# ishine/zerovox.cpp

Measured on AMD Instinct MI355X. Metric: audio-seconds/wall-second (xRT) end-to-end phoneme->22.05 kHz wav, higher is better.
Workload: dtype f16*f16->f32 (MFMA) convs, f32 (MFMA) attention/linear, f32 activations

## Files before the change

zerovox.cpp_amd/csrc/conv_gemm.hip:

```cpp
#include "kernels.h"
#include "knobs.h"
#include "mfma_common.h"

namespace zv
{

__device__ __forceinline__ int gemm_groups_dev(int Cout_p) { return ((Cout_p + 31) >> 5) >> 3; }

__device__ __forceinline__ int conv_gemm_units_dev(int Cin_p, int K)
{
    const int full = Cin_p >> 8, rem = Cin_p & 255;
    return K * (full * 4 + ((rem + 63) >> 6));
}

size_t conv_gemm_weight_halfs(int Cin_p, int Cout_p, int K)
{
    return (size_t)conv_gemm_tiles(Cout_p) * conv_gemm_units(Cin_p, K) * 2048;
}

typedef unsigned int u32x4s __attribute__((ext_vector_type(4)));
__device__ __forceinline__ void dma_piece(u32x4s rsrc, unsigned lds_base, unsigned voff)
{
    unsigned keep;
    asm volatile("s_mov_b32 %0, m0\n\ts_mov_b32 m0, %1\n\ts_nop 4\n\tbuffer_load_dwordx4 %2, %3, 0 offen lds\n\ts_mov_b32 m0, %0"
                 : "=&s"(keep)
                 : "s"(lds_base), "v"(voff), "s"(rsrc)
                 : "memory");
}

__device__ __forceinline__ u32x4s make_rsrc(const void *base, unsigned bytes)
{
    const uint64_t a = (uint64_t)base;
    u32x4s r;
    r[0] = __builtin_amdgcn_readfirstlane((unsigned)a);
    r[1] = __builtin_amdgcn_readfirstlane((unsigned)(a >> 32) & 0xFFFFu);
    r[2] = __builtin_amdgcn_readfirstlane(bytes);
    r[3] = 0x00020000u;
    return r;
}

void pack_conv_weight_gemm(const uint16_t *w, int K, int IC, int OC, int Cin_p, int Cout_p, uint16_t *dst)
{
    const int ng = conv_gemm_groups(Cout_p), nu = conv_gemm_units(Cin_p, K), ntk = conv_gemm_tiles(Cout_p);
    size_t gbase = 0;
    for (int g = 0; g < ng; g++)
    {
        const int ntg = (g == ng - 1) ? ntk - 8 * g : 8;
        int u = 0;
        for (int c0 = 0; c0 < Cin_p; c0 += 256)
        {
            const int nsub = (std::min(256, Cin_p - c0) + 63) / 64;
            for (int tap = 0; tap < K; tap++)
                for (int sub = 0; sub < nsub; sub++, u++)
                    for (int hf = 0; hf < 2; hf++)
                        for (int nt = 0; nt < ntg; nt++)
                            for (int wt = 0; wt < 2; wt++)
                            {
                                uint16_t *d = dst + gbase + ((((size_t)u * 2 + hf) * ntg + nt) * 2 + wt) * 512;
                                for (int lane = 0; lane < 64; lane++)
                                    for (int j = 0; j < 8; j++)
                                    {
                                        const int oc = (g * 8 + nt) * 32 + 2 * (lane & 15) + wt;
                                        const int ic = c0 + sub * 64 + hf * 32 + 8 * (lane >> 4) + j;
                                        d[lane * 8 + j] = (oc < OC && ic < IC) ? w[((size_t)oc * IC + ic) * K + tap] : (uint16_t)0;
                                    }
                            }
        }
        gbase += (size_t)nu * 4 * ntg * 512;
    }
}

template <bool EXTRA>
__device__ __forceinline__ void conv_gemm_body(const ConvJobs &jobs, const int g, const int rt)
{
    constexpr int BM = 256, UNIT = 32768;
    constexpr int ntg = EXTRA ? 9 : 8;
    constexpr int AH = 16384, BH = ntg * 2048;
    constexpr int SLOT = AH + 18432;
    const ConvJob &J = jobs.j[0];
    const int useg = rt / jobs.tps;
    const Seg sg = seg_at(jobs.segs, useg);
    const int L = sg.rows * jobs.rate;
    const int m0 = (rt - useg * jobs.tps) * BM;
    if (m0 >= L) return;
    const size_t row0 = (size_t)sg.row0 * jobs.rate;

    extern __shared__ __attribute__((aligned(1024))) char smem[];
    const unsigned lds0 = (unsigned)(uintptr_t)smem;
    const int tid = threadIdx.x, lane = tid & 63;
    const int wave = __builtin_amdgcn_readfirstlane(tid >> 6);
    const int wm = wave >> 2, wn = wave & 3;
    const int lc = lane & 15, lg = lane >> 4;
    const int K = J.K, dil = J.dil, Cin_p = J.Cin_p, ldx = J.ldx;
    const int nunits = conv_gemm_units_dev(Cin_p, K), nhalf = 2 * nunits;
    constexpr int bunit = ntg * 4096;

    const u32x4s rs_a = make_rsrc((const _Float16 *)J.x0 + row0 * ldx, (unsigned)((size_t)L * ldx * 2));
    const u32x4s rs_b = make_rsrc((const char *)J.w8 + (size_t)g * nunits * UNIT, (unsigned)((size_t)nunits * bunit));

    int a_voff[2];
#pragma unroll
    for (int i = 0; i < 2; i++)
    {
        const int row = (wave * 2 + i) * 16 + (lane >> 2);
        const int piece = (lane & 3) ^ ((row >> 1) & 3);
        a_voff[i] = ((m0 - J.pad + row) * ldx + piece * 8) * 2;
    }

    int uc0 = 0, utap = 0, usub = 0, unsub = (min(256, Cin_p) + 63) >> 6, uh = 0;
    unsigned i_abase = 0;
    int i_aoff = 0, i_boff = 0;
    auto issue_begin = [&](int h) {
        i_abase = lds0 + (h & 3) * SLOT;
        i_aoff = (utap * dil * ldx + uc0 + usub * 64 + uh * 32) * 2;
        i_boff = (h >> 1) * bunit + (h & 1) * BH;
        if (++uh == 2)
        {
            uh = 0;
            if (++usub == unsub)
            {
                usub = 0;
                if (++utap == K)
                {
                    utap = 0;
                    uc0 += 256;
                    unsub = (min(256, Cin_p - uc0) + 63) >> 6;
                }
            }
        }
    };
    auto issue_pa = [&](int i) { dma_piece(rs_a, i_abase + (wave * 2 + i) * 1024, (unsigned)(a_voff[i] + i_aoff)); };
    auto issue_pb = [&](int i) { dma_piece(rs_b, i_abase + AH + (wave * 2 + i) * 1024, (unsigned)(i_boff + (wave * 2 + i) * 1024 + lane * 16)); };
    auto issue_part = [&](int i) {
        issue_pa(i);
        issue_pb(i);
    };
    auto issue_x = [&]() {
        if (EXTRA && wave < 2) dma_piece(rs_b, i_abase + AH + (16 + wave) * 1024, (unsigned)(i_boff + (16 + wave) * 1024 + lane * 16));
    };
    const bool five = EXTRA && wave < 2;

    const int swz = (lc >> 1) & 3;
    const int a_rd = (wm * 128 + lc) * 64 + ((lg ^ swz) << 4);
    const int ax_rd = (wave * 32 + lc) * 64 + ((lg ^ swz) << 4);
    const int b_rd = AH + wn * 4096 + lane * 16;

    floatx4 acc[8][4];
    floatx4 accx[2][2];
    if (wave >= 4) __builtin_amdgcn_s_setprio(1);
#pragma unroll
    for (int h = 0; h < 3; h++)
        if (h < nhalf)
        {
            issue_begin(h);
            issue_part(0);
            issue_part(1);
            issue_x();
        }
    half8 aA[4], bb[4], axA, bxb[2];
#define ZV_G16_READ0(hn)                                                                                          \
    {                                                                                                             \
        const char *nb_ = smem + ((hn) & 3) * SLOT;                                                               \
        _Pragma("unroll") for (int tm = 0; tm < 4; tm++) aA[tm] = *(const half8 *)(nb_ + a_rd + tm * 1024);       \
        _Pragma("unroll") for (int tn = 0; tn < 4; tn++) bb[tn] = *(const half8 *)(nb_ + b_rd + tn * 1024);       \
        if constexpr (EXTRA)                                                                                      \
        {                                                                                                         \
            axA = *(const half8 *)(nb_ + ax_rd);                                                                  \
            bxb[0] = *(const half8 *)(nb_ + AH + 16 * 1024 + lane * 16);                                          \
            bxb[1] = *(const half8 *)(nb_ + AH + 17 * 1024 + lane * 16);                                          \
        }                                                                                                         \
    }
    {
        if (nhalf > 2)
        {
            if (five) asm volatile("s_waitcnt vmcnt(5)" ::: "memory");
            else asm volatile("s_waitcnt vmcnt(4)" ::: "memory");
        }
        else
            asm volatile("s_waitcnt vmcnt(0)" ::: "memory");
        __syncthreads();
        ZV_G16_READ0(0)
    }
    const floatx4 zero4 = {0.f, 0.f, 0.f, 0.f};
    for (int h = 0; h < nhalf; h++)
    {
        if (h > 0)
        {
            if (h + 2 < nhalf)
            {
                if (five) asm volatile("s_waitcnt vmcnt(5)" ::: "memory");
                else asm volatile("s_waitcnt vmcnt(4)" ::: "memory");
            }
            else
                asm volatile("s_waitcnt vmcnt(0)" ::: "memory");
            __syncthreads();
        }
// ... 128 lines not shown
                    v0 = lrelu(v0, J.oslope);
                    v1 = lrelu(v1, J.oslope);
                }
                outv[0][hf][i] = v0;
                outv[1][hf][i] = v1;
                if (t < L)
                {
                    const float2v o = {v0, v1};
                    __builtin_nontemporal_store(o, (float2v *)(out + (size_t)t * J.ldo + oc));
                }
            }
        if (J.stat_part && oc < J.stat_C && blk * 32 < L)
        {
#pragma unroll
            for (int ch = 0; ch < 2; ch++)
            {
                double s1 = 0.0, s2 = 0.0;
#pragma unroll
                for (int st = 0; st < 4; st++)
                {
                    if (st)
                    {
                        s1 = __shfl_xor(s1, 32, 64);
                        s2 = __shfl_xor(s2, 32, 64);
                    }
                    if ((lg >> 1) == (st & 1))
#pragma unroll
                        for (int i = 0; i < 4; i++)
                        {
                            const int t = t_first + 16 * (st >> 1) + 4 * lg + i;
                            const double x = (t < L) ? (double)outv[ch][st >> 1][i] : 0.0;
                            s1 += x;
                            s2 += x * x;
                        }
                }
                s1 += __shfl_xor(s1, 16, 64);
                s2 += __shfl_xor(s2, 16, 64);
                if (lg == 2) *(double2 *)(J.stat_part + (((size_t)useg * J.stat_nblk + blk) * J.stat_C + oc + ch) * 2) = make_double2(s1, s2);
            }
        }
    };
    const int tbase = m0 + wm * 128;
#pragma unroll
    for (int p = 0; p < 2; p++)
#pragma unroll
        for (int b4 = 0; b4 < 4; b4++)
            finish_block(acc[2 * b4][2 * p], acc[2 * b4][2 * p + 1], acc[2 * b4 + 1][2 * p], acc[2 * b4 + 1][2 * p + 1], tbase + b4 * 32,
                         ((g * 8 + wn * 2 + p) << 5) + 2 * lc, (m0 >> 5) + wm * 4 + b4);
    if constexpr (EXTRA)
        finish_block(accx[0][0], accx[0][1], accx[1][0], accx[1][1], m0 + wave * 32, ((g * 8 + 8) << 5) + 2 * lc, (m0 >> 5) + wave);
}

__global__ __launch_bounds__(512, 2) void conv_gemm_kernel(const ConvJobs jobs)
{
    const ConvJob &J = jobs.j[0];
    const int ng = (gemm_groups_dev(J.Cout_p));
    const int rts = jobs.tps * jobs.segs.nseg;
    int g, rt;
    if (jobs.order == 2 && ng > 1)
    {
        if ((int)blockIdx.x < rts) { g = ng - 1; rt = blockIdx.x; }
        else { const int b2 = blockIdx.x - rts; g = b2 % (ng - 1); rt = b2 / (ng - 1); }
    }
    else
    {
        g = blockIdx.x % ng;
        rt = blockIdx.x / ng;
    }
    if (rt >= rts) return;
    const bool ninth = g == ng - 1 && ((J.Cout_p + 31) >> 5) - 8 * ng == 1;
    if (ninth)
        conv_gemm_body<true>(jobs, g, rt);
    else
        conv_gemm_body<false>(jobs, g, rt);
}

hipError_t launch_conv_gemm(hipStream_t s, const ConvJob &job, const Segs &segs, int rate)
{
    const ConvGemmPlan p = conv_gemm_plan(job.Cout_p, ConvCall{1, segs.nseg, segs.max_rows, rate, 0, 0});
    if (job.stat_part && job.stat_nblk * 32 < segs.max_rows * rate) return hipErrorInvalidValue;
    ConvJobs js;
    js.j[0] = job;
    js.j[0].dbg = diag_bits();
    for (int i = 1; i < CONV_MAX_JOBS; i++) js.j[i] = js.j[0];
    js.segs = segs;
    js.rate = rate;
    js.nt_begin = 0;
    js.order = p.order;
    js.tps = p.tps;
    return launch_lds(conv_gemm_kernel, dim3(p.gx, 1, 1), dim3(p.threads), p.lds_bytes, s, js);
}

}
```

zerovox.cpp_amd/csrc/conv_plan.h:

```cpp
#pragma once

#include <stddef.h>

#include "conv_xcd.h"
#include "knobs.h"
#include "tile_deal.h"

namespace zv
{

constexpr long BATCH_ROWS = 16384;
inline bool batch_switch(int value, bool picked_by_itself) { return value != 0 && (value == 2 || picked_by_itself); }
inline bool batch_rows(long rows) { return rows >= BATCH_ROWS; }

constexpr size_t LDS_PER_WG = 160 * 1024;
constexpr size_t LDS_TWO_WGS = 80 * 1024;
constexpr size_t LDS_DEFAULT = 64 * 1024;

inline int plan_round_up(int x, int a) { return (x + a - 1) / a * a; }

inline int &conv_packed_utts()
{
    static thread_local int n = 0;
    return n;
}
struct ConvPackedUtts
{
    int saved;
    explicit ConvPackedUtts(int n) : saved(conv_packed_utts()) { conv_packed_utts() = n; }
    ~ConvPackedUtts() { conv_packed_utts() = saved; }
    ConvPackedUtts(const ConvPackedUtts &) = delete;
    ConvPackedUtts &operator=(const ConvPackedUtts &) = delete;
};

struct ConvCall
{
    int njobs, nseg, max_rows, rate, n_cu, nt_begin;
    int nutt = conv_packed_utts();
};
inline bool conv_call_is_batch(const ConvCall &c) { return c.nseg > 1 || c.nutt > 1; }

inline int conv_gemm_groups(int Cout_p) { return ((Cout_p + 31) / 32) / 8; }
inline int conv_gemm_tiles(int Cout_p)
{
    const int nt = (Cout_p + 31) / 32, ng = nt / 8;
    return ng * 8 + ((nt - ng * 8 == 1 && ng >= 1) ? 1 : 0);
}
inline int conv_gemm_units(int Cin_p, int K)
{
    int n = 0;
    for (int c0 = 0; c0 < Cin_p; c0 += 256) n += K * (((Cin_p - c0 < 256 ? Cin_p - c0 : 256) + 63) / 64);
    return n;
}

enum ConvPrologue : int
{
    PRO_RAW_F16 = 0,
    PRO_ACT = 1,
    PRO_NORM_ACT = 2,
    PRO_MELNORM = 3,
    PRO_SUM3_ACT = 4,
    PRO_SCALE_ACT = 5
};

#ifndef ZV_SINGLE_LW
#define ZV_SINGLE_LW 4
#endif
#ifndef ZV_CONV_BATCH_ROUTE
#define ZV_CONV_BATCH_ROUTE 1
#endif

struct ConvDesc
{
    int  K, dil, pad, Cin_p, Cout_p, ck, pro, ldx;
    bool has_w8, out_f16, has_res, has_stat, eact, three_inputs;
};

inline bool conv_gemm_takes(const ConvDesc &j, const ConvCall &c)
{
    const long rows = (long)c.max_rows * c.rate * c.nseg;
    return batch_switch(knob(ZV_CONV_GEMM), batch_rows(rows)) && j.has_w8 && j.pro == PRO_RAW_F16 && j.Cin_p >= 128 &&
           conv_gemm_groups(j.Cout_p) >= 1 && !j.out_f16 && (j.ldx & 7) == 0;
}

struct ConvGemmPlan
{
    int    order, tps, gx, threads;
    size_t lds_bytes;
};
inline ConvGemmPlan conv_gemm_plan(int Cout_p, const ConvCall &c)
{
    ConvGemmPlan p{};
    p.order = knob(ZV_GEMM_ORDER);
    p.tps = (c.max_rows * c.rate + 255) / 256;
    const int ng = conv_gemm_groups(Cout_p), rts = p.tps * c.nseg;
    p.gx = (p.order == 1 && (ng == 1 || ng == 2 || ng == 4)) ? plan_round_up(rts, 8 / ng) * ng : rts * ng;
    p.threads = 512;
    p.lds_bytes = 4 * (16384 + 18432);
    return p;
}

inline bool conv_stream_ok(const ConvDesc &j, const ConvCall &c)
{
    return c.njobs == 1 && c.nt_begin == 0 && (j.pro == PRO_ACT || j.pro == PRO_SCALE_ACT) && j.K == 3 && j.dil == 1 && j.pad == 1 &&
           (j.Cin_p == 64 || j.Cin_p == 128) && j.ck == j.Cin_p && (j.ldx & 3) == 0 && !j.has_res && !j.has_stat && !j.eact && !j.out_f16 &&
           !j.three_inputs;
}

inline bool conv_tiled_exists(int MT, int WN, int NT)
{
    return (NT == 1 && (MT == 1 || MT == 2 || MT == 4) && (WN == 1 || WN == 2 || WN == 4)) || (NT == 2 && MT == 2 && WN == 4);
}

enum ConvForm { CONV_STREAM, CONV_LOADER, CONV_TILED };
struct ConvPlan
{
    bool     valid;
    ConvForm form;
    int      MT, WN, NT;
    int      strip, nkc;
    int      tps;
    int      gx, gy, gz, threads;
    size_t   lds_bytes;
    int      tile_bytes;
    int      xcd_nx, xcd_ny, xcd_spread;
    int      warm;
};

inline bool conv_plan_tiles(ConvPlan &p, bool loader, int MT, int WN, int NT, int Lmax, int ntiles, int halo, int ck, int dmax, const ConvCall &c)
{
    const int BM = 32 * MT * (4 / WN);
    p.form = loader ? CONV_LOADER : CONV_TILED;
    p.MT = MT, p.WN = WN, p.NT = NT;
    p.tps = (Lmax + BM - 1) / BM;
    p.gx = p.tps * c.nseg, p.gy = (ntiles + WN * NT - 1) / (WN * NT), p.gz = c.njobs;
// ... 272 lines not shown
```

zerovox.cpp_amd/csrc/kernels.h:

```cpp
#pragma once

#include <hip/hip_runtime.h>
#include <stdint.h>

#include "conv_plan.h"
#include "voc_plan.h"
#include "stage_plan.h"
#include "level.h"

#ifdef ZV_DIAG
#define ZV_DBGBITS(x) (x)
#else
#define ZV_DBGBITS(x) 0
#endif

namespace zv
{

__host__ __device__ static inline int round_up(int x, int a) { return (x + a - 1) / a * a; }

struct Seg
{
    int32_t row0, rows;
    int32_t aux;
    int32_t pad;
};
struct Segs
{
    const Seg *tab;
    int        nseg;
    int        max_rows;
    Seg        one;
};
__host__ __device__ static inline Seg seg_at(const Segs &s, int u)
{
    Seg g = s.tab ? s.tab[u] : s.one;
#if defined(__HIP_DEVICE_COMPILE__)
    g.row0 = __builtin_amdgcn_readfirstlane(g.row0);
    g.rows = __builtin_amdgcn_readfirstlane(g.rows);
    g.aux = __builtin_amdgcn_readfirstlane(g.aux);
#endif
    return g;
}
static inline Segs segs_single(int rows, int aux = 0)
{
    Segs s;
    s.tab = nullptr;
    s.nseg = 1;
    s.max_rows = rows;
    s.one.row0 = 0;
    s.one.rows = rows;
    s.one.aux = aux;
    s.one.pad = 0;
    return s;
}


struct ConvJob
{
    const void  *x0, *x1, *x2;
    int          ldx;
    int          pro;
    float        slope, pscale;
    const float *pa, *pb;
    const float *pstat;
    int          L, Cin_p, Cout_p, K, dil, pad;
    int          ck;
    const void  *w;
    const void  *w8;
    const float *bias;
    const float *res;
    int          ldres;
    float        escale;
    int          eact;
    float        oslope;
    int          out_f16;
    void        *out;
    int          ldo;
    int          dbg;
    int          pstat_seg, pab_seg;
    double      *stat_part;
    int          stat_nblk, stat_C;
};

constexpr int CONV_MAX_JOBS = 4;
struct ConvJobs
{
    ConvJob j[CONV_MAX_JOBS];
    Segs    segs;
    int     rate;
    int     tps;
    int     nt_begin;
    int     order;
    int     tile_bytes;
    int     xcd_ny, xcd_nx;
    int     xcd_spread;
    int     warm;
#ifdef ZV_STAMPS
    unsigned long long *stamp;
#endif
};

size_t packed_conv_weight_halfs(int Cin_p, int Cout_p, int K);
int    conv_pick_ck(int Cin_p, int ck_max = 0);
void   pack_conv_weight(const uint16_t *w, int K, int IC, int OC, int Cin_p, int Cout_p, int ck, uint16_t *dst);
size_t conv_gemm_weight_halfs(int Cin_p, int Cout_p, int K);
void   pack_conv_weight_gemm(const uint16_t *w, int K, int IC, int OC, int Cin_p, int Cout_p, uint16_t *dst);
hipError_t launch_conv(hipStream_t s, const ConvJob *jobs, int njobs, int n_cu, const Segs &segs, int rate);

struct PairJob
{
    const float *y;
    float       *out;
    const void  *w1, *w2;
    const void  *w1r, *w2r;
    const float *b1, *b2;
    int          L, Cp, K, dil;
    float        slope;
    int          dbg;
    const float *sum_in;
    float       *sum_out;
};
constexpr int PAIR_MAX_JOBS = 3;
struct PairJobs
{
    PairJob j[PAIR_MAX_JOBS];
    Segs    segs;
    int     rate;
    int     njobs, kmax;
    int     deal_c;
#ifdef ZV_STAMPS
    unsigned long long *stamp;
#endif
    float  *merge_out;
    int     ring_off;
};
size_t     pair_weight_halfs(int Cp, int K);
void       pack_pair_weight(const uint16_t *w, int K, int C, int Cp, uint16_t *dst);
size_t     pair_weight16_halfs(int Cp, int K);
void       pack_pair_weight16(const uint16_t *w, int K, int C, int Cp, uint16_t *dst, bool conv2_layout);
size_t     pair_ring_weight_halfs(int Cp, int K);
void       pack_pair_weight_ring(const uint16_t *w, int K, int C, int Cp, uint16_t *dst, bool conv2_layout);
hipError_t launch_pair(hipStream_t s, const PairJob *jobs, int njobs, int n_cu, const Segs &segs, int rate, float *merge_out = nullptr);

struct TripleJob
{
    const float *y;
    float       *out;
    const void  *w1[TRIPLE_MAX_DIL], *w2[TRIPLE_MAX_DIL];
    const void  *w1x[TRIPLE_MAX_DIL], *w2x[TRIPLE_MAX_DIL];
    const float *b1[TRIPLE_MAX_DIL], *b2[TRIPLE_MAX_DIL];
    int          dil[TRIPLE_MAX_DIL];
// ... 106 lines not shown
```

zerovox.cpp_amd/csrc/knobs.h:

```cpp
#pragma once

namespace zv
{

#define ZV_KNOB_LIST(X)                                                                                                               \
    X(ZV_NO_FUSE, 0)                                                                  \
    X(ZV_NO_TRIPLE, 0)                                                                          \
    X(ZV_FUSE256, 0)                                                \
    X(ZV_NO_MERGE, 0)                                                               \
    X(ZV_MERGE_ALWAYS, 0)                 \
    X(ZV_MERGE_SEQ, 1)          \
    X(ZV_MERGE_MAXC, 256)                                  \
    X(ZV_TAIL_GROUPS, 8)                                                        \
    X(ZV_ARENA_FILL, 0)                                         \
    X(ZV_DEC_PREPASS, -1)                                      \
    X(ZV_CONV_MT, 0)                                                              \
    X(ZV_CONV_NT, 0)                                                     \
    X(ZV_CONV_SINGLE, 1)                                    \
    X(ZV_CONV_GEMM, 1)                  \
    X(ZV_CONV_STREAM, 1)        \
    X(ZV_VOC_RUNS, 1)           \
    X(ZV_DEC_RUNS, 1)           \
    X(ZV_DEC_PACK, 1)           \
    X(ZV_UP_GEMM, 1)           \
    X(ZV_GEMM_ORDER, 2)         \
    X(ZV_PAIR_MT, 0)                                                                  \
    X(ZV_CONV_XCD, 1)           \
    X(ZV_CONV_WARM, 1)          \
    X(ZV_LINEAR_MERGED, 1)      \
    X(ZV_BLOCK64, 3)            \
    X(ZV_PAIR64_RING, 1)               \
    X(ZV_TRIPLE_V2, 1)                               \
    X(ZV_TRIPLE_DB, 1)                                                                     \
    X(ZV_TRIPLE_INTERLEAVE, 1)                                                               \
    X(ZV_ATT_SCALAR, 0)                                                                               \
    X(ZV_ATT_MFMA, 0)                                                          \
    X(ZV_LN_TAIL, 1)

#ifdef ZV_DIAG
#define ZV_KNOB_LIST_DIAG(X)                                                                                                          \
    X(ZV_DBG, 0)                                                                       \
    X(ZV_LDS_PAD, 0)            \
    X(ZV_STAMP_CP, 0)                               \
    X(ZV_STAMP_CONV, 0)                                    \
    X(ZV_STAMP_CIN, 0)
#else
#define ZV_KNOB_LIST_DIAG(X)
#endif

enum Knob : int
{
#define ZV_KNOB_ENUM(n, d) n,
    ZV_KNOB_LIST(ZV_KNOB_ENUM)
    ZV_KNOB_LIST_DIAG(ZV_KNOB_ENUM)
#undef ZV_KNOB_ENUM
    ZV_KNOB_COUNT
};

int         knob(Knob k);
bool        knob_set(const char *name, int value);
void        knob_reset();
bool        knob_get(const char *name, int *value);
unsigned    knob_epoch();
const char *knob_name(int k);
#ifdef ZV_DIAG
inline int diag_bits() { return knob(ZV_DBG); }
#else
inline int diag_bits() { return 0; }
#endif

}
```

zerovox.cpp_amd/csrc/model.cpp:

```cpp
#include "schedule.h"

#include <algorithm>

namespace zv
{

Model::~Model()
{
    hipSetDevice(device);
    for (Lane &l : lanes_) hipStreamSynchronize(l.stream);
    drop_graphs();
    prof_clear();
    for (void *p : allocs_) hipFree(p);
    for (hipEvent_t e : batch_events_)
        if (e) hipEventDestroy(e);
    for (Lane &l : lanes_)
    {
        if (l.copy_stream) hipStreamSynchronize(l.copy_stream);
        if (l.arena.base) hipFree(l.arena.base);
        if (l.io) hipFree(l.io);
        if (l.pinned) hipHostFree(l.pinned);
        for (hipEvent_t e : l.tail_events) hipEventDestroy(e);
        if (l.copy_stream) hipStreamDestroy(l.copy_stream);
        if (l.stream) hipStreamDestroy(l.stream);
// ... 120 lines not shown
    ZV_HIP(hipStreamSynchronize(stream()));
    drop_graphs();
    DeviceArena &ar = lane().arena;
    if (ar.base) hipFree(ar.base);
    ar = DeviceArena();
    lane().runs_tab = nullptr;
    lane().runs_n = 0;
    void *p = nullptr;
    if (hipMalloc(&p, bytes) != hipSuccess) fail(ZV_ERR_OOM, "hipMalloc(%zu) for the activation arena failed", bytes);
    const int fill = knob(ZV_ARENA_FILL);
    ZV_HIP(hipMemsetAsync(p, fill, bytes, stream()));
    ar = DeviceArena{(char *)p, bytes, 0};
}

void Model::reserve(uint32_t max_phonemes, uint32_t max_frames) { reserve_batch(Batch::single(std::max(1u, max_phonemes), std::max(1u, max_frames), 1)); }

void Model::reserve_batch(const Batch &b) { arena_require(arena_bytes_for(b)); }


void Model::prof_clear()
{
    for (auto &p : prof)
    {
        hipEventDestroy(p.e0);
        hipEventDestroy(p.e1);
    }
    prof.clear();
}

void Model::tick(hipEvent_t *e0)
{
    *e0 = nullptr;
    if (!profiling || in_group_) return;
    ZV_HIP(hipEventCreate(e0));
    ZV_HIP(hipEventRecord(*e0, stream()));
}

void Model::tock(hipEvent_t e0, const char *name, double bytes, double flops)
{
    if (!profiling) return;
    if (in_group_)
    {
        group_bytes_ += bytes;
        group_flops_ += flops;
        group_n_++;
        return;
    }
    hipEvent_t e1;
    ZV_HIP(hipEventCreate(&e1));
    ZV_HIP(hipEventRecord(e1, stream()));
    prof.push_back({name, e0, e1, bytes, flops, group_n_ > 0 ? group_n_ : 1});
}

void Model::group_begin()
{
    if (!profiling) return;
    ZV_HIP(hipEventCreate(&group_e0_));
    ZV_HIP(hipEventRecord(group_e0_, stream()));
    in_group_ = true;
    group_bytes_ = group_flops_ = 0.0;
    group_n_ = 0;
}

void Model::group_end(const char *name)
{
    if (!profiling || !in_group_) return;
    in_group_ = false;
    tock(group_e0_, name, group_bytes_, group_flops_);
    group_n_ = 0;
}

ConvJob Model::job(const ConvW &w) const
{
    ConvJob j;
    memset(&j, 0, sizeof(j));
    j.Cin_p = w.Cin_p;
    j.Cout_p = w.Cout_p;
    j.K = w.K;
    j.dil = 1;
    j.pad = (w.K - 1) / 2;
    j.ck = w.ck;
    j.w = w.w;
    j.w8 = w.w8;
    j.bias = w.bias;
    j.pro = PRO_ACT;
    j.slope = 1.0f;
    j.pscale = 1.0f;
    j.escale = 1.0f;
    j.ldx = w.Cin_p;
    j.ldo = w.Cout_p;
    return j;
}

void Model::dbg_inject(void *dev, int ld, int cols, size_t rows)
{
    ZV_HIP(hipMemcpy2DAsync(dev, (size_t)ld * 4, dbg_layer.x, (size_t)cols * 4, (size_t)cols * 4, rows, hipMemcpyHostToDevice, stream()));
}

void Model::dbg_extract(const void *dev, int ld, int cols, size_t rows)
{
    ZV_HIP(hipMemcpy2DAsync(dbg_layer.out, (size_t)cols * 4, dev, (size_t)ld * 4, (size_t)cols * 4, rows, hipMemcpyDeviceToHost, stream()));
    ZV_HIP(hipStreamSynchronize(stream()));
    dbg_layer.done = true;
}

void Model::conv(const ConvJob *jobs, int n, const Segs &segs, int rate, const char *name, double bytes, double flops)
{
    ZV_LAUNCH(name, bytes, flops, launch_conv(stream(), jobs, n, n_cu, segs, rate));
}

void Model::drop_graphs()
{
    sync_all_lanes();
    for (auto &g : graphs_)
        if (g.exec) hipGraphExecDestroy(g.exec);
    graphs_.clear();
}

template <typename F> void Model::run_captured(int kind, const Batch &b, const void *const (&key)[CapturedGraph::NKEY], F &&enqueue)
{
    for (auto &g : graphs_)
        if (g.kind == kind && g.epoch == knob_epoch() && b.same_schedule(g.b) && memcmp(g.p, key, sizeof(key)) == 0)
        {
            ZV_HIP(hipGraphLaunch(g.exec, stream()));
            lane().runs_tab = g.runs_tab;
            lane().runs_n = g.runs_n;
            return;
        }
    reserve_batch(b);
    hipGraph_t graph = nullptr;
    lane().runs_tab = nullptr;
    lane().runs_n = 0;
    ZV_HIP(hipStreamBeginCapture(stream(), hipStreamCaptureModeThreadLocal));
    try
    {
        enqueue();
    }
    catch (...)
    {
        hipStreamEndCapture(stream(), &graph);
        if (graph) hipGraphDestroy(graph);
        throw;
    }
    ZV_HIP(hipStreamEndCapture(stream(), &graph));
    CapturedGraph cg;
    cg.kind = kind;
    cg.epoch = knob_epoch();
    cg.b = b;
    memcpy(cg.p, key, sizeof(key));
    cg.runs_tab = lane().runs_tab;
    cg.runs_n = lane().runs_n;
    hipError_t e = hipGraphInstantiate(&cg.exec, graph, nullptr, nullptr, 0);
    hipGraphDestroy(graph);
    if (e != hipSuccess) fail(ZV_ERR_DEVICE, "hipGraphInstantiate failed: %s", hipGetErrorString(e));
    if (graphs_.size() >= 16)
    {
        ZV_HIP(hipStreamSynchronize(stream()));
        drop_graphs();
    }
    graphs_.push_back(cg);
    ZV_HIP(hipGraphLaunch(cg.exec, stream()));
}

void Model::chain_dev(const Batch &b, const int32_t *d_ids, const int32_t *d_puncts, const float *d_styles, float *d_hidden,
                      float *d_mel, float *d_wav, int32_t *d_nframes, const void *h2d_src, void *h2d_dst, size_t h2d_bytes, int voc_part)
{
// ... 21 lines not shown
```

zerovox.cpp_amd/csrc/model.h:

```cpp
#pragma once

#include <cstdint>
#include <cstring>
#include <string>
#include <vector>

#include "common.h"
#include "gguf_reader.h"
#include "kernels.h"

namespace zv
{

struct ConvW
{
    void  *w = nullptr;
    void  *w8 = nullptr;
    float *bias = nullptr;
    int    K = 0, Cin = 0, Cout = 0, Cin_p = 0, Cout_p = 0, ck = 0;
};

struct DeviceArena
{
    char  *base = nullptr;
    size_t cap = 0, used = 0;
    static size_t align(size_t off) { return (off + 255) & ~(size_t)255; }
    static DeviceArena counter() { return DeviceArena{nullptr, SIZE_MAX, 0}; }
    void  *take(size_t bytes)
    {
        const size_t a = align(used);
        if (a + bytes > cap) fail(ZV_ERR_OOM, "device arena overflow (%zu + %zu > %zu)", a, bytes, cap);
        used = a + bytes;
        return base ? base + a : nullptr;
    }
    template <typename T> T *take_n(size_t n) { return (T *)take(n * sizeof(T)); }
};

struct ProfEntry
{
    const char *name;
    hipEvent_t  e0, e1;
    double      bytes, flops;
    int         launches;
};

struct Batch
{
    int        nseg = 1;
    int        n_max = 0, t_max = 0;
    int        n_real = 0;
    size_t     n_rows = 0, t_rows = 0;
    const Seg *d_tok = nullptr, *d_frm = nullptr;
    Seg        tok1{0, 0, 0, 0}, frm1{0, 0, 0, 0};
    const float *d_ctl = nullptr;
    const float *d_pctl = nullptr;
    int32_t *d_cum = nullptr;
    Seg *d_frm_live = nullptr;
    Seg *d_dec_runs = nullptr;
    bool has_targets = false;
    const float   *d_vol = nullptr;
    LevelRow      *d_levels = nullptr;
    const int32_t *d_nframes = nullptr;

    static Batch single(uint32_t N, uint32_t T, uint32_t num_phonemes)
    {
        Batch b;
        b.n_max = (int)N;
        b.n_real = (int)N;
        b.t_max = (int)T;
        b.n_rows = N;
        b.t_rows = T;
        b.tok1 = Seg{0, (int32_t)N, (int32_t)num_phonemes, 0};
        b.frm1 = Seg{0, (int32_t)T, 0, 0};
        return b;
    }
    Segs tokens() const { return Segs{d_tok, nseg, n_max, tok1}; }
    Segs tokens_merged() const { return d_tok ? Segs{d_tok + nseg, 1, (int)n_rows, tok1} : tokens(); }
    Segs frames_cap() const { return Segs{d_frm, nseg, t_max, frm1}; }
    Segs frames() const { return d_frm_live ? Segs{d_frm_live, nseg, t_max, frm1} : frames_cap(); }
    bool same_schedule(const Batch &o) const
    {
        return nseg == o.nseg && n_max == o.n_max && t_max == o.t_max && n_rows == o.n_rows && t_rows == o.t_rows && d_tok == o.d_tok &&
               d_frm == o.d_frm && (d_tok || memcmp(&tok1, &o.tok1, sizeof(Seg)) == 0) && (d_frm || memcmp(&frm1, &o.frm1, sizeof(Seg)) == 0) &&
               d_ctl == o.d_ctl && d_pctl == o.d_pctl && d_cum == o.d_cum && d_frm_live == o.d_frm_live && has_targets == o.has_targets &&
               d_dec_runs == o.d_dec_runs && d_vol == o.d_vol && d_levels == o.d_levels && d_nframes == o.d_nframes;
    }
};

struct CapturedGraph
{
    static constexpr int NKEY = 8;
    int            kind = 0;
    unsigned       epoch = 0;
    Batch          b;
    const void    *p[NKEY] = {};
    hipGraphExec_t exec = nullptr;
    const Seg     *runs_tab = nullptr;
    int            runs_n = 0;
};

class Model
{
  public:
    Model(const std::string &gguf_path, int device);
    ~Model();

    zv_hparams hp{};
    int        device = 0;
    int        n_cu = 256;
    hipStream_t stream() const { return lanes_[cur_lane_].stream; }

    void vocode_dev(const Batch &b, const float *d_mel, float *d_wav);
    void vocode_group(const Batch &b, const float *d_mel, float *d_wav, int part = 0, int seg0 = 0);
    void vocode_tail(const Batch &b, const float *d_mel, float *d_wav, int g0, int cnt);
    hipStream_t copy_stream();
    hipEvent_t  tail_event(int i);
    static constexpr int BATCH_RING = 64;
    uint64_t    next_batch_seq() { return batch_seq_++; }
    uint64_t    batch_seq() const { return batch_seq_; }
    hipEvent_t  batch_event(uint64_t seq, int which);
    void decode_dev(const Batch &b, const float *d_hidden, const float *d_styles, float *d_mel);
    struct EncoderTaps
    {
        float   *features = nullptr, *logdur = nullptr, *pitch = nullptr, *energy = nullptr;
        int32_t *pitch_bucket = nullptr, *energy_bucket = nullptr, *cum = nullptr;
    };
    EncoderTaps encode_dev(const Batch &b, const int32_t *d_ids, const int32_t *d_puncts, const float *d_styles,
                           float *d_hidden, int32_t *d_nframes);

    struct DebugLayer
    {
        int          kind = -1, index = 0;
        const float *x = nullptr;
        float       *out = nullptr;
        bool         done = false;
    } dbg_layer;

    uint32_t max_phonemes() const { return (uint32_t)enc_.posenc_rows; }
    void reserve(uint32_t max_phonemes, uint32_t max_frames);
    void reserve_batch(const Batch &b);
    int  voc_stage_rate(int stage) const;
    int  voc_stage_channels(int stage) const;
    uint32_t max_frames_per_utterance() const;
    int wemb_rows() const { return enc_.wemb_rows; }
    int pemb_rows() const { return enc_.pemb_rows; }
    uint32_t vocoder_halo_frames() const;
    bool voc_runs_off = false;
    bool voc_runs_on(const Batch &b) const;
    const Seg *voc_runs_last(int *n) { *n = lane().runs_n; return lane().runs_tab; }
    DecPlan dec_plan(const Batch &b) const
    {
        return zv::dec_plan(b.nseg, b.t_max, b.t_rows, b.d_frm_live != nullptr, dbg_layer.kind >= 0, b.d_dec_runs != nullptr);
    }
    int  dec_reach_frames() const;
    void sync();

    void select_lane(int i);
    int  selected_lane() const { return cur_lane_; }
    void sync_all_lanes();
    void poison_lane(int i, int byte, size_t filled[3]);

    void *io_scratch(size_t bytes);
    void *pinned_scratch(size_t bytes);

    bool graph_mode = false;
    void vocode_dev_graph(const Batch &b, const float *d_mel, float *d_wav);
    void chain_dev(const Batch &b, const int32_t *d_ids, const int32_t *d_puncts, const float *d_styles, float *d_hidden,
                   float *d_mel, float *d_wav, int32_t *d_nframes, const void *h2d_src = nullptr, void *h2d_dst = nullptr,
                   size_t h2d_bytes = 0, int voc_part = 0);

    bool profiling = false;
    std::vector<ProfEntry> prof;
    void prof_clear();

    uint32_t E() const { return hp.emb_dim + hp.punct_emb_dim; }
    void debug_layernorm(int index, uint32_t n);

  private:
    std::vector<void *> allocs_;
    void  *dev_alloc(size_t bytes);
    float *upload_f32(const GgufTensor &t, int pad_to = 0, float pad_value = 0.f);
    float *upload_vec(const GgufFile &g, const std::string &name, int expect_n, int pad_to = 0, float pad_value = 0.f);
    ConvW  load_conv(const GgufFile &g, const std::string &wname, const std::string &bname, int expect_cin = -1, bool gemm_pack = false);
    ConvW  load_upsample(const GgufFile &g, int idx, int stride, int expect_cin);

    struct ResPair { ConvW c1, c2; void *p1 = nullptr, *p2 = nullptr, *r1 = nullptr, *r2 = nullptr, *x1 = nullptr, *x2 = nullptr; };
    struct Voc
    {
        float *mean = nullptr, *scale = nullptr;
        ConvW  in_conv;
        int    n_up = 0;
        int    scales[8] = {0};
        ConvW  ups[8];
        int    n_rb = 0, n_dil = 3;
        int    dil[8] = {1, 3, 5};
        std::vector<ResPair> pairs;
        uint16_t *out_w = nullptr;
        float  out_b = 0.f;
        int    out_K = 0, out_C = 0;
    } voc_;
    VocGeom voc_geom_{};
    VocCall voc_call(const Batch &b) const;
    TripleJob block_job(const ResPair *rp, int n_dil, bool ring, const float *y, float *out) const;
    struct DilPairJobs { ConvJob c1, c2; PairJob p; };
    DilPairJobs pair_jobs(const ResPair &rp, int dil, const float *yin, float *yout, _Float16 *xt, float *y) const;

    struct DecBlk
    {
        ConvW  conv1, conv2, sc;
        bool   learned_sc = false;
        int    cin = 0, cout = 0;
        float *n1w = nullptr, *n1b = nullptr, *n2w = nullptr, *n2b = nullptr;
        int    g1 = 0, g2 = 0;
    };
    struct Dec
    {
        DecBlk enc[2], dec[5];
        ConvW  asr0, to_out;
        float *asr1w = nullptr, *asr1b = nullptr;
        float *fcW = nullptr, *fcB = nullptr, *fcExtra = nullptr;
        int    fc_out = 0;
        int    R = 64, M = 80;
    } dec_;

    struct EncLayer
    {
        float *qkvW = nullptr, *qkvB = nullptr, *fcW = nullptr, *fcB = nullptr;
        float *ln1w = nullptr, *ln1b = nullptr, *ln2w = nullptr, *ln2b = nullptr;
        ConvW  w1, w2;
    };
    struct VarPred
    {
        ConvW  c1, c2;
        float *l1w = nullptr, *l1b = nullptr, *l2w = nullptr, *l2b = nullptr, *lw = nullptr, *lb = nullptr;
        int    V = 0;
    };
    struct Enc
    {
        float *wemb = nullptr, *pemb = nullptr, *posenc = nullptr, *pitch_emb = nullptr, *energy_emb = nullptr;
        int    posenc_rows = 0, wemb_rows = 0, pemb_rows = 0;
        std::vector<EncLayer> layers;
        VarPred dur, pitch, energy;
    } enc_;

    struct VocLayout
    {
        float *c0;
        struct Stage { float *ub, *y[3]; _Float16 *xt[3]; } st[8];
        void *level_slab;
        float *mel_c; int32_t *eq; Seg *runs;
    };
    size_t level_slab_entries(const Batch &b) const;
    struct DecLayout
    {
        int    nblk, hs, ss;
        int    rows, nblk_all;
        float *h, *st_x, *st_t, *st_y, *st_a, *cat, *t1, *sc, *x0, *xa, *asr_t;
        double *part_t, *part_o; _Float16 *xa16, *t16, *xr16;
        float *mel_c;
    };
    struct EncLayout { int Vp; float *x, *y, *qkv, *o, *f, *va, *vb; _Float16 *hh; EncoderTaps t; };
    VocLayout voc_layout(DeviceArena &a, const Batch &b) const;
    DecLayout dec_layout(DeviceArena &a, const Batch &b) const;
    EncLayout enc_layout(DeviceArena &a, const Batch &b) const;
    static constexpr size_t ARENA_TAIL = (size_t)1 << 20;
    size_t arena_bytes_for(const Batch &b) const;
// ... 43 lines not shown
```

zerovox.cpp_amd/csrc/model_load.cpp:

```cpp
#include "model.h"
#include "knobs.h"

#include <algorithm>

namespace zv
{

static const char *KV_PREFIX = "zerovox-resnet-fs2-styletts.";

void *Model::dev_alloc(size_t bytes)
{
    void *p = nullptr;
    if (bytes == 0) bytes = 16;
    if (hipMalloc(&p, bytes) != hipSuccess) fail(ZV_ERR_OOM, "hipMalloc(%zu) failed", bytes);
    allocs_.push_back(p);
    return p;
}

float *Model::upload_f32(const GgufTensor &t, int pad_to, float pad_value)
{
    if (t.type != GGML_F32) fail(ZV_ERR_SHAPE, "tensor %s: expected f32", t.name.c_str());
    const size_t n = (size_t)t.nelements();
    const size_t np = pad_to > 0 ? (size_t)std::max<int64_t>(pad_to, (int64_t)n) : n;
    std::vector<float> h(np + 64, pad_value);
    memcpy(h.data(), t.data, n * sizeof(float));
    float *d = (float *)dev_alloc(h.size() * sizeof(float));
    ZV_HIP(hipMemcpy(d, h.data(), h.size() * sizeof(float), hipMemcpyHostToDevice));
    return d;
}

float *Model::upload_vec(const GgufFile &g, const std::string &name, int expect_n, int pad_to, float pad_value)
{
    const GgufTensor &t = g.get(name);
    if (t.nelements() != expect_n) fail(ZV_ERR_SHAPE, "tensor %s: expected %d elements, found %lld", name.c_str(), expect_n, (long long)t.nelements());
    return upload_f32(t, pad_to, pad_value);
}

ConvW Model::load_conv(const GgufFile &g, const std::string &wname, const std::string &bname, int expect_cin, bool gemm_pack)
{
    const GgufTensor &w = g.get(wname);
    if (w.type != GGML_F16) fail(ZV_ERR_SHAPE, "tensor %s: conv weights must be f16", wname.c_str());
    ConvW c;
    c.K = (int)w.ne[0];
    c.Cin = (int)w.ne[1];
    c.Cout = (int)w.ne[2];
    if (expect_cin >= 0 && c.Cin != expect_cin) fail(ZV_ERR_SHAPE, "tensor %s: expected %d input channels, found %d", wname.c_str(), expect_cin, c.Cin);
    if ((c.K & 1) == 0) fail(ZV_ERR_SHAPE, "tensor %s: even kernel size %d is not a 'same' conv", wname.c_str(), c.K);
    c.Cin_p = round_up(c.Cin, 16);
    c.Cout_p = round_up(c.Cout, 16);
    c.ck = conv_pick_ck(c.Cin_p);
    std::vector<uint16_t> packed(packed_conv_weight_halfs(c.Cin_p, c.Cout_p, c.K));
    pack_conv_weight((const uint16_t *)w.data, c.K, c.Cin, c.Cout, c.Cin_p, c.Cout_p, c.ck, packed.data());
    c.w = dev_alloc(packed.size() * 2 + 32768);
    ZV_HIP(hipMemcpy(c.w, packed.data(), packed.size() * 2, hipMemcpyHostToDevice));
    if (gemm_pack && c.Cin_p >= 256 && conv_gemm_groups(c.Cout_p) >= 1)
    {
        std::vector<uint16_t> p8(conv_gemm_weight_halfs(c.Cin_p, c.Cout_p, c.K));
        pack_conv_weight_gemm((const uint16_t *)w.data, c.K, c.Cin, c.Cout, c.Cin_p, c.Cout_p, p8.data());
        c.w8 = dev_alloc(p8.size() * 2);
        ZV_HIP(hipMemcpy(c.w8, p8.data(), p8.size() * 2, hipMemcpyHostToDevice));
    }
    if (!bname.empty())
    {
        const GgufTensor &b = g.get(bname);
        if (b.type != GGML_F32 || b.nelements() != c.Cout) fail(ZV_ERR_SHAPE, "tensor %s: expected f32[%d]", bname.c_str(), c.Cout);
        c.bias = upload_f32(b, round_up(c.Cout_p, 32), 0.f);
    }
    return c;
}

ConvW Model::load_upsample(const GgufFile &g, int idx, int stride, int expect_cin)
{
    char nm[96];
    snprintf(nm, sizeof(nm), "_meldec.upsamples.%d.1.w", idx);
    const GgufTensor &w = g.get(nm);
    if (w.type != GGML_F16) fail(ZV_ERR_SHAPE, "tensor %s: conv weights must be f16", nm);
    const int K = (int)w.ne[0], IC = (int)w.ne[1], OC = (int)w.ne[2];
    if (IC != expect_cin) fail(ZV_ERR_SHAPE, "tensor %s: expected %d input channels, found %d", nm, expect_cin, IC);
    const int s = stride;
    const int p = s / 2 + s % 2, op = s % 2;
    const int off = (K - 1) - p;
    if (2 * off + op + 1 - (K - 1) != s) fail(ZV_ERR_SHAPE, "tensor %s: kernel %d / stride %d do not give L*s outputs", nm, K, s);
    int dmin = 0, dmax = 0;
    for (int r = 0; r < s; r++)
        for (int k = 0; k < K; k++)
            if ((k - off + r) % s == 0)
            {
                const int d = (k - off + r) / s;
                dmin = std::min(dmin, d);
                dmax = std::max(dmax, d);
            }
    const int nd = std::max(-dmin, dmax);
    ConvW c;
    c.K = 2 * nd + 1;
    c.Cin = IC;
    c.Cin_p = round_up(IC, 16);
    const int OCp = round_up(OC, 16);
    c.Cout = s * OCp;
    c.Cout_p = s * OCp;
    const bool gemm_pack = c.Cin_p >= 128 && (c.Cin_p & 63) == 0 && conv_gemm_groups(c.Cout_p) >= 1 && c.K * c.Cin_p >= 768;
    c.ck = conv_pick_ck(c.Cin_p, gemm_pack ? 256 : 128);
    std::vector<uint16_t> v((size_t)c.Cout * IC * c.K, 0);
    const uint16_t *src = (const uint16_t *)w.data;
    for (int r = 0; r < s; r++)
        for (int oc = 0; oc < OC; oc++)
            for (int ic = 0; ic < IC; ic++)
                for (int tp = 0; tp < c.K; tp++)
                {
                    const int k = off - r + (tp - nd) * s;
                    if (k >= 0 && k < K) v[((size_t)(r * OCp + oc) * IC + ic) * c.K + tp] = src[((size_t)oc * IC + ic) * K + k];
                }
    std::vector<uint16_t> packed(packed_conv_weight_halfs(c.Cin_p, c.Cout_p, c.K));
    pack_conv_weight(v.data(), c.K, IC, c.Cout, c.Cin_p, c.Cout_p, c.ck, packed.data());
    c.w = dev_alloc(packed.size() * 2 + 32768);
    ZV_HIP(hipMemcpy(c.w, packed.data(), packed.size() * 2, hipMemcpyHostToDevice));
    if (gemm_pack)
    {
        std::vector<uint16_t> p8(conv_gemm_weight_halfs(c.Cin_p, c.Cout_p, c.K));
        pack_conv_weight_gemm(v.data(), c.K, IC, c.Cout, c.Cin_p, c.Cout_p, p8.data());
        c.w8 = dev_alloc(p8.size() * 2);
        ZV_HIP(hipMemcpy(c.w8, p8.data(), p8.size() * 2, hipMemcpyHostToDevice));
    }
    snprintf(nm, sizeof(nm), "_meldec.upsamples.%d.1.b", idx);
    const GgufTensor &b = g.get(nm);
    if (b.type != GGML_F32 || b.nelements() != OC) fail(ZV_ERR_SHAPE, "tensor %s: expected f32[%d]", nm, OC);
    std::vector<float> hb(round_up(c.Cout_p, 32) + 64, 0.f);
    for (int r = 0; r < s; r++) memcpy(hb.data() + (size_t)r * OCp, b.data, (size_t)OC * 4);
    c.bias = (float *)dev_alloc(hb.size() * 4);
    ZV_HIP(hipMemcpy(c.bias, hb.data(), hb.size() * 4, hipMemcpyHostToDevice));
    return c;
}

Model::Model(const std::string &path, int dev) : device(dev)
{
    int ndev = 0;
    if (hipGetDeviceCount(&ndev) != hipSuccess || ndev <= 0) fail(ZV_ERR_DEVICE, "no HIP device available");
    if (dev < 0 || dev >= ndev) fail(ZV_ERR_ARG, "device %d out of range (%d devices)", dev, ndev);
    ZV_HIP(hipSetDevice(dev));
    hipDeviceProp_t prop;
    ZV_HIP(hipGetDeviceProperties(&prop, dev));
    if (strncmp(prop.gcnArchName, "gfx950", 6) != 0) fail(ZV_ERR_DEVICE, "device %d is %s; this library is built for gfx950 only", dev, prop.gcnArchName);
    n_cu = prop.multiProcessorCount;
    lanes_.resize(1);
    ZV_HIP(hipStreamCreateWithFlags(&lanes_[0].stream, hipStreamNonBlocking));

    GgufFile g;
    g.open(path);
    auto kv = [&](const char *k) { return g.get_u32(std::string(KV_PREFIX) + k); };
    hp.max_seq_len = kv("max_seq_len");
    hp.emb_dim = kv("emb_dim");
    hp.punct_emb_dim = kv("punct_emb_dim");
    hp.decoder_n_head = kv("decoder.n_head");
    hp.conv_filter_size = kv("decoder.conv_filter_size");
    hp.conv_kernel_size[0] = kv("decoder.conv_kernel_size.0");
    hp.conv_kernel_size[1] = kv("decoder.conv_kernel_size.1");
    hp.encoder_layer = kv("encoder.layer");
    hp.encoder_head = kv("encoder.head");
    hp.encoder_vp_filter_size = kv("encoder.vp_filter_size");
    hp.encoder_vp_kernel_size = kv("encoder.vp_kernel_size");
    hp.encoder_ve_n_bins = kv("encoder.ve_n_bins");
    hp.audio_sampling_rate = kv("audio.sampling_rate");
    hp.audio_num_mels = kv("audio.num_mels");
    hp.audio_hop_size = kv("audio.hop_size");

    const int Ed = (int)E();
    if (Ed % 16) fail(ZV_ERR_SHAPE, "emb_dim + punct_emb_dim = %d must be a multiple of 16", Ed);
    if (hp.audio_num_mels % 16) fail(ZV_ERR_SHAPE, "num_mels = %u must be a multiple of 16", hp.audio_num_mels);
    if (hp.encoder_head == 0 || Ed % hp.encoder_head) fail(ZV_ERR_SHAPE, "encoder.head = %u does not divide %d", hp.encoder_head, Ed);
    if (hp.encoder_vp_kernel_size != 3) fail(ZV_ERR_SHAPE, "vp_kernel_size = %u: the reference pads the second predictor conv with a literal 1 (src/fs2encoder.cpp:417), only 3 is a 'same' conv", hp.encoder_vp_kernel_size);
    char nm[128], nb[128];

    const int M = (int)hp.audio_num_mels;
    voc_.mean = upload_vec(g, "hifigan.mean", M);
    voc_.scale = upload_vec(g, "hifigan.scale", M, 0, 1.f);
    voc_.in_conv = load_conv(g, "_meldec.input_conv.w", "_meldec.input_conv.b", M);
    if (voc_.in_conv.K != 7) fail(ZV_ERR_SHAPE, "tensor _meldec.input_conv.w: kernel size %d, the reference pads for 7", voc_.in_conv.K);
    int C = voc_.in_conv.Cout;
    hp.voc_channels = C;
    int n_up = 0;
    while (n_up < 8)
    {
        snprintf(nm, sizeof(nm), "_meldec.upsamples.%d.1.w", n_up);
        if (!g.find(nm)) break;
        n_up++;
    }
    if (n_up == 0) fail(ZV_ERR_MISSING, "tensor '_meldec.upsamples.0.1.w' not found");
    static const int REF_SCALES[4] = {5, 5, 4, 3};
    if (n_up != 4) fail(ZV_ERR_SHAPE, "tensor _meldec.upsamples.%d.1.w: %s; the reference runs 4 upsample stages, the file has %d", std::min(n_up, 4),
                          n_up < 4 ? "missing" : "unexpected", n_up);
    int hop = 1;
    voc_.n_up = n_up;
    hp.voc_num_upsamples = n_up;
    int n_blocks = 0;
    while (true)
    {
        snprintf(nm, sizeof(nm), "_meldec.blocks.%d.convs1.0.1.w", n_blocks);
        if (!g.find(nm)) break;
        n_blocks++;
    }
    if (n_blocks == 0 || n_blocks % n_up) fail(ZV_ERR_SHAPE, "%d residual blocks do not divide over %d upsample stages", n_blocks, n_up);
    voc_.n_rb = n_blocks / n_up;
    if (voc_.n_rb != 3) fail(ZV_ERR_SHAPE, "num_resblocks = %d: the schedule (like the reference caller) is built for 3", voc_.n_rb);
    hp.voc_num_resblocks = voc_.n_rb;
    for (int i = 0; i < n_up; i++)
// ... 257 lines not shown
```

Before: 34910.

## Skip all-zero weight slices in GEMM conv via per-group live unit table

At load time, the packed GEMM conv weights are scanned per output group, and a table lists only the K-slices (tap, channel half) with nonzero weights. The kernel then walks this table instead of the full tap/channel loop, skipping loads and MFMAs for zero slices. This mainly targets polyphase upsample convs, whose folded taps are often zero. It adds a small per-step table read and a default-on knob.

```diff
diff --git a/zerovox.cpp_amd/csrc/conv_gemm.hip b/zerovox.cpp_amd/csrc/conv_gemm.hip
--- a/zerovox.cpp_amd/csrc/conv_gemm.hip
+++ b/zerovox.cpp_amd/csrc/conv_gemm.hip
@@ -19,6 +19,8 @@
 }
 
 typedef unsigned int u32x4s __attribute__((ext_vector_type(4)));
+typedef unsigned int u32x2s __attribute__((ext_vector_type(2)));
+typedef __attribute__((address_space(4))) u32x2s LiveEntry;
 __device__ __forceinline__ void dma_piece(u32x4s rsrc, unsigned lds_base, unsigned voff)
 {
     unsigned keep;
@@ -92,7 +94,16 @@
     const int wm = wave >> 2, wn = wave & 3;
     const int lc = lane & 15, lg = lane >> 4;
     const int K = J.K, dil = J.dil, Cin_p = J.Cin_p, ldx = J.ldx;
-    const int nunits = conv_gemm_units_dev(Cin_p, K), nhalf = 2 * nunits;
+    const int nunits = conv_gemm_units_dev(Cin_p, K);
+    const LiveEntry *live = nullptr;
+    int nhalf = 2 * nunits;
+    if (J.live8)
+    {
+        const LiveEntry *tab = (const LiveEntry *)J.live8;
+        const u32x2s hd = tab[g];
+        live = tab + hd[0];
+        nhalf = (int)hd[1];
+    }
     constexpr int bunit = ntg * 4096;
 
     const u32x4s rs_a = make_rsrc((const _Float16 *)J.x0 + row0 * ldx, (unsigned)((size_t)L * ldx * 2));
@@ -107,11 +118,21 @@
         a_voff[i] = ((m0 - J.pad + row) * ldx + piece * 8) * 2;
     }
 
+    u32x2s live_nx = {0u, 0u};
+    if (live) live_nx = live[0];
     int uc0 = 0, utap = 0, usub = 0, unsub = (min(256, Cin_p) + 63) >> 6, uh = 0;
     unsigned i_abase = 0;
     int i_aoff = 0, i_boff = 0;
     auto issue_begin = [&](int h) {
         i_abase = lds0 + (h & 3) * SLOT;
+        if (live)
+        {
+            const u32x2s e = live_nx;
+            live_nx = live[h + 1];
+            i_aoff = ((int)(e[0] & 255u) * dil * ldx + (int)(e[0] >> 8)) * 2;
+            i_boff = (int)e[1];
+            return;
+        }
         i_aoff = (utap * dil * ldx + uc0 + usub * 64 + uh * 32) * 2;
         i_boff = (h >> 1) * bunit + (h & 1) * BH;
         if (++uh == 2)
@@ -406,6 +427,7 @@
     ConvJobs js;
     js.j[0] = job;
     js.j[0].dbg = diag_bits();
+    if (!conv_zskip_on()) js.j[0].live8 = nullptr;
     for (int i = 1; i < CONV_MAX_JOBS; i++) js.j[i] = js.j[0];
     js.segs = segs;
     js.rate = rate;
diff --git a/zerovox.cpp_amd/csrc/conv_plan.h b/zerovox.cpp_amd/csrc/conv_plan.h
--- a/zerovox.cpp_amd/csrc/conv_plan.h
+++ b/zerovox.cpp_amd/csrc/conv_plan.h
@@ -1,6 +1,9 @@
 #pragma once
 
 #include <stddef.h>
+#include <stdint.h>
+
+#include <vector>
 
 #include "conv_xcd.h"
 #include "knobs.h"
@@ -51,6 +54,75 @@
     int n = 0;
     for (int c0 = 0; c0 < Cin_p; c0 += 256) n += K * (((Cin_p - c0 < 256 ? Cin_p - c0 : 256) + 63) / 64);
     return n;
+}
+
+inline bool conv_zskip_on() { return knob(ZV_CONV_ZSKIP) != 0; }
+inline bool conv_halfs_all_zero(const uint16_t *p, size_t n)
+{
+    for (size_t i = 0; i < n; i++)
+        if (p[i] & 0x7FFFu) return false;
+    return true;
+}
+
+struct ConvGemmLive
+{
+    uint32_t tap_ch;
+    uint32_t boff;
+};
+constexpr int CONV_GEMM_LIVE_MAX_TAPS = 256;
+inline std::vector<ConvGemmLive> conv_gemm_full_walk(int Cin_p, int K, int ntg)
+{
+    std::vector<ConvGemmLive> v;
+    uint32_t h = 0;
+    for (int c0 = 0; c0 < Cin_p; c0 += 256)
+    {
+        const int nsub = ((Cin_p - c0 < 256 ? Cin_p - c0 : 256) + 63) / 64;
+        for (int tap = 0; tap < K; tap++)
+            for (int sub = 0; sub < nsub; sub++)
+                for (int hf = 0; hf < 2; hf++, h++)
+                    v.push_back(ConvGemmLive{(uint32_t)tap | (uint32_t)(c0 + sub * 64 + hf * 32) << 8, h * (uint32_t)ntg * 2048u});
+    }
+    return v;
+}
+inline std::vector<ConvGemmLive> conv_gemm_live_map(const uint16_t *w8, int Cin_p, int Cout_p, int K)
+{
+    std::vector<ConvGemmLive> t;
+    const int ng = conv_gemm_groups(Cout_p), nu = conv_gemm_units(Cin_p, K), ntk = conv_gemm_tiles(Cout_p);
+    if (ng < 1 || K > CONV_GEMM_LIVE_MAX_TAPS) return t;
+    t.resize(ng);
+    size_t gbase = 0;
+    for (int g = 0; g < ng; g++)
+    {
+        const int ntg = (g == ng - 1) ? ntk - 8 * g : 8;
+        const std::vector<ConvGemmLive> full = conv_gemm_full_walk(Cin_p, K, ntg);
+        const uint32_t first = (uint32_t)t.size();
+        for (const ConvGemmLive &e : full)
+            if (!conv_halfs_all_zero(w8 + gbase + e.boff / 2, (size_t)ntg * 1024)) t.push_back(e);
+        if (t.size() == first) t.push_back(full[0]);
+        t[g] = ConvGemmLive{first, (uint32_t)t.size() - first};
+        const ConvGemmLive last = t.back();
+        t.push_back(last);
+        gbase += (size_t)nu * 2 * ntg * 1024;
+    }
+    return t;
+}
+
+constexpr int CONV_TILE_TAPS_MAX = 32;
+inline std::vector<uint32_t> conv_tile_live_taps(const uint16_t *w, int Cin_p, int Cout_p, int K, int ck)
+{
+    std::vector<uint32_t> m;
+    if (K > CONV_TILE_TAPS_MAX) return m;
+    const int ntiles = (Cout_p + 31) / 32, nicb = Cin_p / 16;
+    m.assign(ntiles, 0u);
+    for (int nt = 0; nt < ntiles; nt++)
+        for (int c0 = 0; c0 < Cin_p; c0 += ck)
+        {
+            const int nkc = ((Cin_p - c0 < ck) ? (Cin_p - c0) : ck) / 16;
+            for (int tap = 0; tap < K; tap++)
+                if (!conv_halfs_all_zero(w + ((size_t)nt * K * nicb + (size_t)K * (c0 / 16) + (size_t)tap * nkc) * 512, (size_t)nkc * 512))
+                    m[nt] |= 1u << tap;
+        }
+    return m;
 }
 
 enum ConvPrologue : int
diff --git a/zerovox.cpp_amd/csrc/kernels.h b/zerovox.cpp_amd/csrc/kernels.h
--- a/zerovox.cpp_amd/csrc/kernels.h
+++ b/zerovox.cpp_amd/csrc/kernels.h
@@ -68,6 +68,7 @@
     int          ck;
     const void  *w;
     const void  *w8;
+    const ConvGemmLive *live8;
     const float *bias;
     const float *res;
     int          ldres;
diff --git a/zerovox.cpp_amd/csrc/knobs.h b/zerovox.cpp_amd/csrc/knobs.h
--- a/zerovox.cpp_amd/csrc/knobs.h
+++ b/zerovox.cpp_amd/csrc/knobs.h
@@ -23,6 +23,7 @@
     X(ZV_DEC_RUNS, 1)           \
     X(ZV_DEC_PACK, 1)           \
     X(ZV_UP_GEMM, 1)           \
+    X(ZV_CONV_ZSKIP, 1)         \
     X(ZV_GEMM_ORDER, 2)         \
     X(ZV_PAIR_MT, 0)                                                                  \
     X(ZV_CONV_XCD, 1)           \
diff --git a/zerovox.cpp_amd/csrc/model.cpp b/zerovox.cpp_amd/csrc/model.cpp
--- a/zerovox.cpp_amd/csrc/model.cpp
+++ b/zerovox.cpp_amd/csrc/model.cpp
@@ -226,6 +226,7 @@
     j.ck = w.ck;
     j.w = w.w;
     j.w8 = w.w8;
+    j.live8 = w.live8;
     j.bias = w.bias;
     j.pro = PRO_ACT;
     j.slope = 1.0f;
diff --git a/zerovox.cpp_amd/csrc/model.h b/zerovox.cpp_amd/csrc/model.h
--- a/zerovox.cpp_amd/csrc/model.h
+++ b/zerovox.cpp_amd/csrc/model.h
@@ -16,6 +16,7 @@
 {
     void  *w = nullptr;
     void  *w8 = nullptr;
+    ConvGemmLive *live8 = nullptr;
     float *bias = nullptr;
     int    K = 0, Cin = 0, Cout = 0, Cin_p = 0, Cout_p = 0, ck = 0;
 };
@@ -182,6 +183,7 @@
     float *upload_f32(const GgufTensor &t, int pad_to = 0, float pad_value = 0.f);
     float *upload_vec(const GgufFile &g, const std::string &name, int expect_n, int pad_to = 0, float pad_value = 0.f);
     ConvW  load_conv(const GgufFile &g, const std::string &wname, const std::string &bname, int expect_cin = -1, bool gemm_pack = false);
+    void   upload_live_map(ConvW &c, const uint16_t *p8);
     ConvW  load_upsample(const GgufFile &g, int idx, int stride, int expect_cin);
 
     struct ResPair { ConvW c1, c2; void *p1 = nullptr, *p2 = nullptr, *r1 = nullptr, *r2 = nullptr, *x1 = nullptr, *x2 = nullptr; };
diff --git a/zerovox.cpp_amd/csrc/model_load.cpp b/zerovox.cpp_amd/csrc/model_load.cpp
--- a/zerovox.cpp_amd/csrc/model_load.cpp
+++ b/zerovox.cpp_amd/csrc/model_load.cpp
@@ -34,6 +34,14 @@
     const GgufTensor &t = g.get(name);
     if (t.nelements() != expect_n) fail(ZV_ERR_SHAPE, "tensor %s: expected %d elements, found %lld", name.c_str(), expect_n, (long long)t.nelements());
     return upload_f32(t, pad_to, pad_value);
+}
+
+void Model::upload_live_map(ConvW &c, const uint16_t *p8)
+{
+    const std::vector<ConvGemmLive> live = conv_gemm_live_map(p8, c.Cin_p, c.Cout_p, c.K);
+    if (live.empty()) return;
+    c.live8 = (ConvGemmLive *)dev_alloc(live.size() * sizeof(ConvGemmLive));
+    ZV_HIP(hipMemcpy(c.live8, live.data(), live.size() * sizeof(ConvGemmLive), hipMemcpyHostToDevice));
 }
 
 ConvW Model::load_conv(const GgufFile &g, const std::string &wname, const std::string &bname, int expect_cin, bool gemm_pack)
@@ -59,6 +67,7 @@
         pack_conv_weight_gemm((const uint16_t *)w.data, c.K, c.Cin, c.Cout, c.Cin_p, c.Cout_p, p8.data());
         c.w8 = dev_alloc(p8.size() * 2);
         ZV_HIP(hipMemcpy(c.w8, p8.data(), p8.size() * 2, hipMemcpyHostToDevice));
+        upload_live_map(c, p8.data());
     }
     if (!bname.empty())
     {
@@ -120,6 +129,7 @@
         pack_conv_weight_gemm(v.data(), c.K, IC, c.Cout, c.Cin_p, c.Cout_p, p8.data());
         c.w8 = dev_alloc(p8.size() * 2);
         ZV_HIP(hipMemcpy(c.w8, p8.data(), p8.size() * 2, hipMemcpyHostToDevice));
+        upload_live_map(c, p8.data());
     }
     snprintf(nm, sizeof(nm), "_meldec.upsamples.%d.1.b", idx);
     const GgufTensor &b = g.get(nm);
```

Result: no change. 35190, median of 6 (+0.8%).
